# bebop/poly

Measured on AMD Instinct MI355X. Metric: mash.Sketch k-mers hashed/s, higher is better.
Workload: dtype u32

## Files before the change

### poly_amd/csrc/mash_sketch.hip

```cpp
#include <hip/hip_runtime.h>

#include <algorithm>

#include "common.h"
#include "host_pipeline.h"
#include "multi_device.h"
#include <memory>
#include <string>
#include <vector>

#ifndef PH_WPE
#define PH_WPE 6
#endif
#ifndef PH_CAPK
#define PH_CAPK 12u
#endif
#ifndef PH_ABL
#define PH_ABL 0
#endif
#ifndef PH_SELBINS
#define PH_SELBINS 0
#endif
#ifndef PH_SEL_ATOMIC
#define PH_SEL_ATOMIC 0
#endif
#ifndef PH_BS_WIN
#define PH_BS_WIN 4
#endif
#ifndef PH_BS_U
#define PH_BS_U 4
#endif
#ifndef PH_SLAB_SIG
#define PH_SLAB_SIG 6u
#endif
#ifndef PH_SLAB_CW
#define PH_SLAB_CW 6u
#endif
#ifndef PH_SLAB_CF
#define PH_SLAB_CF 0u
#endif
#ifndef PH_SLAB_WPE
#define PH_SLAB_WPE PH_WPE
#endif

namespace polyhip {
namespace k1 {

constexpr int THREADS = 256;
constexpr int WAVES = THREADS / 64;
#ifndef PH_WTW
#define PH_WTW 512
#endif
constexpr int WTW = PH_WTW;
constexpr int TW = WTW * WAVES;
constexpr int GROUPS = WTW / (4 * 64);
constexpr int NB = 2048;
constexpr uint32_t MARK0 = 0xFFFFFFFFu, MARK1 = 0u;
constexpr int GBATCH = 32;
constexpr uint32_t WL_POSITIONAL = 0x80000000u;
constexpr uint32_t C1 = 0xcc9e2d51u, C2 = 0x1b873593u;

__device__ __forceinline__ uint32_t rotl32(uint32_t x, int r) { return (x << r) | (x >> (32 - r)); }

__device__ __forceinline__ uint32_t premix(uint32_t k)
{
    k *= C1;
    k = rotl32(k, 15);
    k *= C2;
    return k;
}

__device__ __forceinline__ uint32_t chain(uint32_t h) { return rotl32(h, 13) * 5u + 0xe6546b64u; }

__device__ __forceinline__ uint32_t fmix32(uint32_t h)
{
    h ^= h >> 16;
    h *= 0x85ebca6bu;
    h ^= h >> 13;
    h *= 0xc2b2ae35u;
    h ^= h >> 16;
    return h;
}

__device__ __forceinline__ uint32_t funnel_bytes(uint32_t hi, uint32_t lo, uint32_t sh)
{
    return __builtin_amdgcn_alignbyte(hi, lo, sh);
}

__device__ __forceinline__ uint32_t wave_incl_scan(uint32_t v)
{
    v += (uint32_t)__builtin_amdgcn_update_dpp(0, (int)v, 0x111, 0xF, 0xF, true);
    v += (uint32_t)__builtin_amdgcn_update_dpp(0, (int)v, 0x112, 0xF, 0xF, true);
    v += (uint32_t)__builtin_amdgcn_update_dpp(0, (int)v, 0x114, 0xF, 0xF, true);
    v += (uint32_t)__builtin_amdgcn_update_dpp(0, (int)v, 0x118, 0xF, 0xF, true);
    v += (uint32_t)__builtin_amdgcn_update_dpp(0, (int)v, 0x142, 0xA, 0xF, false);
    v += (uint32_t)__builtin_amdgcn_update_dpp(0, (int)v, 0x143, 0xC, 0xF, false);
    return v;
}

struct Smem {
    uint32_t *seqb;
    uint32_t *P;
    uint32_t *cand;
    uint32_t *binned;
    uint32_t *misc;
    uint32_t *lut;
};

constexpr uint32_t BIG_BIN = 32;
constexpr uint32_t BIG_LIST_CAP = 512;

template <class Emit>
__device__ __attribute__((noinline)) void rank_big_bins(const uint32_t *__restrict__ binned, const uint32_t *__restrict__ bins,
                                              const uint32_t *__restrict__ biglist, uint32_t nbig, uint32_t s, Emit emit)
{
    const int lane = threadIdx.x & 63, wave = threadIdx.x >> 6;
    const uint64_t below = (1ull << lane) - 1ull;
    for (uint32_t q = wave; q < nbig; q += WAVES) {
        const uint32_t b = biglist[q];
        const uint32_t st = b ? bins[b - 1] : 0u, en = bins[b];
        uint32_t base = st, lastv = 0;
        bool first = true;
        while (base < s && base < en) {
            uint32_t m = 0xFFFFFFFFu;
            bool has = false;
            for (uint32_t x = st + lane; x < en; x += 64) {
                const uint32_t o = binned[x];
                if (first || o > lastv) {
                    m = min(m, o);
                    has = true;
                }
            }
            if (__ballot(has) == 0ull)
                break;
#pragma unroll
            for (int d = 32; d >= 1; d >>= 1)
                m = min(m, (uint32_t)__shfl_xor((int)m, d, 64));
            for (uint32_t x0 = st; x0 < en; x0 += 64) {
                const uint32_t x = x0 + lane;
                const bool eq = x < en && binned[x] == m;
                const uint64_t mask = __ballot(eq);
                const uint32_t pos = base + (uint32_t)__builtin_popcountll(mask & below);
                if (eq && pos < s)
                    emit(pos, m);
                base += (uint32_t)__builtin_popcountll(mask);
            }
            lastv = m;
            first = false;
        }
    }
}

template <class ForEach>
__device__ uint32_t bottom_s(const Smem &sm, uint32_t s, uint32_t tau, uint32_t binned_cap, bool keep_partial,
                             ForEach for_each)
{
    const int tid = threadIdx.x;
    uint32_t *bins = sm.P;
    const int sig = 32 - __builtin_clz(tau | 1u);
    const int shift = sig > 11 ? sig - 11 : 0;
    __syncthreads();

    for (int b = tid; b < NB; b += THREADS)
        bins[b] = 0;
    if (tid == 0)
        sm.misc[8] = 0;
    __syncthreads();
    for_each([&](uint32_t h) {
        if (h <= tau)
            atomicAdd(&bins[h >> shift], 1u);
    });
    __syncthreads();

    {
        uint32_t v[8], sum = 0;
#pragma unroll
        for (int i = 0; i < 8; ++i) {
            v[i] = bins[8 * tid + i];
            sum += v[i];
        }
        uint32_t incl = sum;
#pragma unroll
        for (int d = 1; d < 64; d <<= 1) {
            uint32_t t = __shfl_up(incl, d, 64);
            if ((tid & 63) >= d)
                incl += t;
        }
        if ((tid & 63) == 63)
            sm.misc[4 + (tid >> 6)] = incl;
        __syncthreads();
        uint32_t run = incl - sum;
        for (int w = 0; w < (tid >> 6); ++w)
            run += sm.misc[4 + w];
#pragma unroll
        for (int i = 0; i < 8; ++i) {
            bins[8 * tid + i] = run;
// ... 188 lines not shown
        }
#pragma unroll
        for (int c = 0; c < 4; ++c)
            h[c] = PH_ABL == 3 ? h[c] : fmix32(h[c]);
        emit(4u * (uint32_t)wq, h);
    }
    wave_sync();
}

template <int KS, bool LOCKSTEP, class Before, class EmitFull, class EmitPart>
__device__ __forceinline__ void run_tiles(const Smem &sm, const uint32_t *__restrict__ gdw, uint32_t gsh,
                                          int64_t gbytes, int64_t nwin, uint32_t k, uint32_t n_seq_dw, uint32_t n_P_w,
                                          Before before, EmitFull emit_full, EmitPart emit_part)
{
    const int wave = threadIdx.x >> 6;
    uint32_t *seqb = sm.seqb + wave * n_seq_dw;
    uint32_t *P = sm.P + wave * n_P_w;
    const int64_t stage_bytes = (int64_t)n_seq_dw * 4 + 4;
    auto is_full = [&](int64_t t0) { return (nwin - t0) >= (int64_t)WTW && t0 + stage_bytes <= gbytes; };
    Stager<KS> st;
    const int64_t first = (int64_t)wave * WTW;
    if (first < nwin)
        st.load(gdw, gsh, gbytes, first, n_seq_dw, is_full(first));
    for (int64_t T0 = 0; T0 < nwin; T0 += TW) {
        if (LOCKSTEP)
            before(T0);
        const int64_t t0 = T0 + first;
        if (t0 >= nwin)
            continue;
        const bool full = is_full(t0);
        st.store(seqb, gdw, gsh, gbytes, t0, n_seq_dw, full);
        wave_sync();
        if (t0 + TW < nwin)
            st.load(gdw, gsh, gbytes, t0 + TW, n_seq_dw, is_full(t0 + TW));
        if (full) {
            tile_compute<KS>(seqb, P, sm.lut, k, [&](uint32_t w0, const uint32_t(&h)[4]) { emit_full(t0, w0, h, 4u); });
        } else {
            const uint32_t wl = (uint32_t)((nwin - t0) < (int64_t)WTW ? (nwin - t0) : (int64_t)WTW);
            tile_compute<KS>(seqb, P, sm.lut, k, [&](uint32_t w0, const uint32_t(&h)[4]) {
                emit_part(t0, w0, h, w0 >= wl ? 0u : (wl - w0 < 4u ? wl - w0 : 4u));
            });
        }
    }
}

__device__ __forceinline__ void append4(uint32_t *__restrict__ counter, uint32_t *__restrict__ cand, uint32_t cap,
                                        const uint32_t (&h)[4], uint32_t nvalid, uint32_t tau)
{
    bool a[4];
    uint64_t m[4];
    uint32_t cnt[4], total = 0;
#pragma unroll
    for (int c = 0; c < 4; ++c) {
        a[c] = (PH_ABL == 4 ? h[c] == 12345u : h[c] <= tau) && (uint32_t)c < nvalid;
        m[c] = __ballot(a[c]);
        cnt[c] = (uint32_t)__popcll(m[c]);
        total += cnt[c];
    }
    if (total == 0)
        return;
    uint32_t base = 0;
    if ((threadIdx.x & 63) == 0)
        base = atomicAdd(counter, total);
    base = __builtin_amdgcn_readfirstlane(base);
#pragma unroll
    for (int c = 0; c < 4; ++c) {
        if (a[c]) {
            const uint32_t idx = base + __builtin_amdgcn_mbcnt_hi((uint32_t)(m[c] >> 32),
                                                                  __builtin_amdgcn_mbcnt_lo((uint32_t)m[c], 0u));
            if (idx < cap)
                cand[idx] = h[c];
        }
        base += cnt[c];
    }
}

constexpr int BSU = PH_BS_U;
constexpr uint32_t BS_MARGIN = (PH_BS_WIN + 3u) & ~3u;
#define BS_SYNC()              \
    do {                       \
        if (PH_ABL != 21)      \
            __syncthreads();   \
    } while (0)
template <bool FIN, bool SELB = false>
__device__ void bottom_s_fast(const Smem &sm, uint32_t s, uint32_t tau, uint32_t C, uint32_t nbf_log2,
                              uint32_t *__restrict__ outp, const uint32_t *__restrict__ src, uint32_t first,
                              uint32_t step, uint32_t cnt, uint32_t *__restrict__ selbins = nullptr)
{
    const int tid = threadIdx.x;
    auto fin = [](uint32_t h) { return FIN ? h ^ (h >> 16) : h; };
    uint32_t *bins = sm.P;
    const uint32_t nbf = 1u << nbf_log2;
    const int sig = 32 - __builtin_clz(tau | 1u);
    const int shift = sig > (int)nbf_log2 ? sig - (int)nbf_log2 : 0;
    uint4 *bins4 = reinterpret_cast<uint4 *>(bins);
    const int q4 = (int)(nbf / (4 * THREADS));
    if (!SELB) {
        for (int q = 0; q < q4; ++q)
            bins4[q4 * tid + q] = make_uint4(0, 0, 0, 0);
        if (tid == 0)
            sm.misc[8] = 0;
    }
    if (PH_BS_WIN) {
        if (tid < PH_BS_WIN)
            sm.binned[-1 - tid] = 0u;
        else if (tid < 2 * PH_BS_WIN)
            sm.binned[C + (uint32_t)tid - PH_BS_WIN] = 0xFFFFFFFFu;
    }
    if (!SELB)
        BS_SYNC();
    if (!SELB) {
        for (uint32_t i0 = first; i0 < cnt; i0 += BSU * step) {
            uint32_t h[BSU];
#pragma unroll
            for (int u = 0; u < BSU; ++u)
                h[u] = i0 + u * step < cnt ? fin(src[i0 + u * step]) : 0u;
#pragma unroll
            for (int u = 0; u < BSU; ++u)
                if (i0 + u * step < cnt)
                    atomicAdd(&bins[h[u] >> shift], 1u);
        }
        BS_SYNC();
    }
    {
        uint4 v[2];
        uint32_t sum = 0;
        uint4 *cnt4 = SELB ? reinterpret_cast<uint4 *>(selbins) : bins4;
        for (int q = 0; q < 2; ++q) {
            v[q] = q < q4 ? cnt4[q4 * tid + q] : make_uint4(0, 0, 0, 0);
            if (SELB && q < q4)
                cnt4[q4 * tid + q] = make_uint4(0, 0, 0, 0);
            sum += v[q].x + v[q].y + v[q].z + v[q].w;
        }
        const uint32_t incl = wave_incl_scan(sum);
        if ((tid & 63) == 63)
            sm.misc[4 + (tid >> 6)] = incl;
        BS_SYNC();
        uint32_t run = incl - sum;
        for (int w = 0; w < (tid >> 6); ++w)
            run += sm.misc[4 + w];
        for (int q = 0; q < 2; ++q) {
            if (q < q4) {
                uint4 o;
                o.x = run;
                o.y = o.x + v[q].x;
                o.z = o.y + v[q].y;
                o.w = o.z + v[q].z;
                run = o.w + v[q].w;
                bins4[q4 * tid + q] = o;
                if (max(max(v[q].x, v[q].y), max(v[q].z, v[q].w)) > BIG_BIN) {
                    const uint32_t cnt4[4] = {v[q].x, v[q].y, v[q].z, v[q].w};
#pragma unroll
                    for (int c = 0; c < 4; ++c)
                        if (cnt4[c] > BIG_BIN) {
                            const uint32_t slot = atomicAdd(&sm.misc[8], 1u);
                            if (slot < BIG_LIST_CAP)
                                sm.seqb[slot] = (uint32_t)(4 * (q4 * tid + q) + c);
                        }
                }
            }
        }
    }
    BS_SYNC();
    for (uint32_t i0 = first; i0 < cnt; i0 += BSU * step) {
        uint32_t h[BSU], at[BSU];
#pragma unroll
        for (int u = 0; u < BSU; ++u)
            h[u] = i0 + u * step < cnt ? fin(src[i0 + u * step]) : 0u;
#pragma unroll
        for (int u = 0; u < BSU; ++u)
            if (i0 + u * step < cnt)
                at[u] = atomicAdd(&bins[h[u] >> shift], 1u);
#pragma unroll
        for (int u = 0; u < BSU; ++u)
            if (i0 + u * step < cnt)
                sm.binned[at[u]] = h[u];
    }
    BS_SYNC();
    const uint32_t nbig = sm.misc[8];
    const bool by_waves = nbig <= BIG_LIST_CAP;
    auto rank_in_bin = [&](uint32_t j, uint32_t hv) {
        const uint32_t b = hv >> shift;
        const uint32_t start = b ? bins[b - 1] : 0u, end = bins[b];
        if (start >= s || (by_waves && end - start > BIG_BIN))
            return;
        uint32_t pos = start;
        for (uint32_t x = start; x < end; ++x) {
            const uint32_t o = sm.binned[x];
            pos += (o < hv) || (o == hv && x < j);
        }
        if (pos < s)
            outp[pos] = hv;
    };
#if PH_BS_WIN
    if (PH_ABL != 22) {
        const uint32_t lim = 1u << shift;
        for (uint32_t j = tid; j < C; j += THREADS) {
            const uint32_t *__restrict__ w = sm.binned + j;
            const uint32_t hv = w[0];
            uint32_t pos = j;
            bool far;
            {
                uint32_t l[PH_BS_WIN], r[PH_BS_WIN];
#pragma unroll
                for (int d = 0; d < PH_BS_WIN; ++d) {
                    l[d] = w[-1 - d];
                    r[d] = w[1 + d];
                }
#pragma unroll
                for (int d = 0; d < PH_BS_WIN; ++d) {
                    pos -= l[d] > hv ? 1u : 0u;
                    pos += r[d] < hv ? 1u : 0u;
                }
                far = ((l[PH_BS_WIN - 1] ^ hv) < lim) | ((r[PH_BS_WIN - 1] ^ hv) < lim);
            }
            if (__builtin_expect(far, 0))
                rank_in_bin(j, hv);
            else if (pos < s)
                outp[pos] = hv;
        }
    }
#else
    for (uint32_t j = tid; j < C; j += THREADS)
        rank_in_bin(j, sm.binned[j]);
#endif
    if (by_waves && nbig)
        rank_big_bins(sm.binned, bins, sm.seqb, nbig, s, [outp](uint32_t pos, uint32_t hv) { outp[pos] = hv; });
}

struct ReadView {
    const uint32_t *gdw;
    uint32_t gsh;
    int64_t gbytes, nwin;
};

__device__ __forceinline__ ReadView view(const uint8_t *__restrict__ seqs, const uint64_t *__restrict__ offs,
                                         uint64_t r, uint32_t k)
{
    ReadView v;
    const uint64_t o0 = offs[r], o1 = offs[r + 1];
    const int64_t n = (int64_t)(o1 - o0);
    v.nwin = n - (int64_t)k;
    v.gsh = (uint32_t)((uintptr_t)(seqs + o0) & 3);
    v.gdw = reinterpret_cast<const uint32_t *>(seqs + o0 - v.gsh);
    v.gbytes = n + v.gsh;
    return v;
}

template <int KS>
__global__ __launch_bounds__(THREADS) __attribute__((amdgpu_waves_per_eu(PH_WPE, 8))) void sketch_fast_kernel(const uint8_t *__restrict__ seqs,
                                                             const uint64_t *__restrict__ offs, uint64_t nseq,
                                                             uint32_t k_rt, uint32_t s, uint32_t *__restrict__ out,
                                                             uint32_t n_seq_dw, uint32_t n_P_w, uint32_t n_P,
                                                             uint32_t capf, uint32_t nbf_log2)
{
    extern __shared__ __attribute__((aligned(16))) uint32_t smem_raw[];
    Smem sm;
    sm.seqb = smem_raw;
    sm.P = sm.seqb + WAVES * n_seq_dw;
    sm.cand = sm.P + n_P;
    sm.binned = sm.cand + capf + BS_MARGIN;
    sm.misc = sm.binned + capf + BS_MARGIN;
    sm.lut = sm.misc + 16;

    const uint32_t k = KS > 0 ? (uint32_t)KS : k_rt;
    const int tid = threadIdx.x;
    sm.lut[tid] = premix((uint32_t)tid) ^ k;
    auto nothing = [](int64_t) {};

    for (uint64_t r = blockIdx.x; r < nseq; r += gridDim.x) {
        const ReadView rv = view(seqs, offs, r, k);
        if (rv.nwin <= 0)
            continue;
        uint32_t *__restrict__ outp = out + r * (uint64_t)s;

        if (rv.nwin < (int64_t)s) {
            __syncthreads();
            auto put = [&](int64_t t0, uint32_t w0, const uint32_t(&h)[4], uint32_t nvalid) {
#pragma unroll
                for (int c = 0; c < 4; ++c)
                    if ((uint32_t)c < nvalid)
                        outp[t0 + w0 + c] = h[c];
            };
            run_tiles<KS, false>(sm, rv.gdw, rv.gsh, rv.gbytes, rv.nwin, k, n_seq_dw, n_P_w, nothing, put, put);
            continue;
        }

        uint32_t tau0 = 0xFFFFFFFFu;
        {
            const uint64_t target = (uint64_t)s + 6ull * (uint64_t)__builtin_sqrtf((float)s) + 16ull;
            if ((int64_t)target < rv.nwin)
                tau0 = (uint32_t)((target << 32) / (uint64_t)rv.nwin);
        }
        bool ok = tau0 != 0xFFFFFFFFu || rv.nwin <= (int64_t)capf;
        __syncthreads();
        if (tid == 0)
            sm.misc[0] = 0;
        __syncthreads();
        uint32_t C = 0;
        if (ok) {
            auto keep = [&](int64_t, uint32_t, const uint32_t(&h)[4], uint32_t nvalid) {
                append4(&sm.misc[0], sm.cand, capf, h, nvalid, tau0);
            };
            run_tiles<KS, false>(sm, rv.gdw, rv.gsh, rv.gbytes, rv.nwin, k, n_seq_dw, n_P_w, nothing, keep, keep);
            __syncthreads();
            C = sm.misc[0];
            ok = C >= s && C <= capf;
        }
        if (ok) {
            if (PH_ABL == 5) {
                for (uint32_t i = tid; i < s; i += THREADS)
                    outp[i] = sm.cand[i];
            } else {
                bottom_s_fast<false>(sm, s, tau0, C, nbf_log2, outp, sm.cand, (uint32_t)tid, THREADS, C);
            }
        } else if (tid == 0) {
            outp[0] = MARK0;
            outp[1] = MARK1;
        }
    }
}

template <int KS> struct Slabs {
    static constexpr int NBLK = KS >> 2, TAIL = KS & 3;
    static constexpr int DUPD = NBLK + 2;
    const uint32_t *__restrict__ gdw;
    uint32_t gsh;
    int64_t gbytes;
    uint32_t *__restrict__ seqb;
    uint32_t *__restrict__ P;
    const uint32_t *__restrict__ lut;
    int lane;

    uint32_t u_inside;
    __device__ __forceinline__ void gload(uint32_t u, uint32_t &lo, uint32_t &hi) const
    {
        const uint32_t *__restrict__ slab = gdw + (uint64_t)u * 64;
        hi = 0u;
        if (__builtin_expect(u < u_inside, 1)) {
            lo = slab[lane];
            if (gsh)
                hi = slab[lane + 1];
        } else {
            const int64_t left = gbytes - (int64_t)u * 256;
            lo = (int64_t)lane * 4 < left ? slab[lane] : 0u;
            if (gsh)
                hi = (int64_t)(lane + 1) * 4 < left ? slab[lane + 1] : 0u;
        }
    }

    template <int PAR> __device__ __forceinline__ void stage(uint32_t lo, uint32_t hi) const
    {
        const uint32_t v = gsh ? funnel_bytes(hi, lo, gsh) : lo;
        seqb[1 + 64 * PAR + lane] = v;
        if (PAR == 0) {
            if (lane < DUPD)
                seqb[129 + lane] = v;
        } else if (lane == 63) {
            seqb[0] = v;
        }
    }

    template <int PAR> __device__ __forceinline__ void premix_unit() const
    {
        const uint32_t d0 = seqb[64 * PAR + lane], d1 = seqb[64 * PAR + lane + 1];
        uint4 p;
        p.x = premix(d0);
        p.y = premix(funnel_bytes(d1, d0, 1));
        p.z = premix(funnel_bytes(d1, d0, 2));
        p.w = premix(funnel_bytes(d1, d0, 3));
        uint4 *P4 = reinterpret_cast<uint4 *>(P);
        if (PAR == 0) {
            P4[(lane + 127) & 127] = p;
            if (lane >= 1 && lane <= NBLK)
                P4[127 + lane] = p;
        } else {
            P4[63 + lane] = p;
        }
    }

    template <int PAR> __device__ __forceinline__ void hash(uint32_t (&h)[4]) const
    {
        const uint4 *b = reinterpret_cast<const uint4 *>(P) + 64 * PAR + lane;
        h[0] = h[1] = h[2] = h[3] = 0u;
#pragma unroll
        for (int j = 0; j < (PH_ABL == 16 ? 1 : NBLK); ++j) {
            const uint4 p = b[j];
            h[0] = chain(h[0] ^ p.x);
            h[1] = chain(h[1] ^ p.y);
            h[2] = chain(h[2] ^ p.z);
            h[3] = chain(h[3] ^ p.w);
        }
        const uint32_t *t = seqb + 1 + 64 * PAR + lane + NBLK;
        if (TAIL == 1) {
            const uint32_t tb = t[0];
            uint32_t off[4];
            const uint32_t two = 2u;
            asm("v_lshlrev_b32_sdwa %0, %1, %2 dst_sel:DWORD dst_unused:UNUSED_PAD src0_sel:DWORD src1_sel:BYTE_0" : "=v"(off[0]) : "v"(two), "v"(tb));
            asm("v_lshlrev_b32_sdwa %0, %1, %2 dst_sel:DWORD dst_unused:UNUSED_PAD src0_sel:DWORD src1_sel:BYTE_1" : "=v"(off[1]) : "v"(two), "v"(tb));
            asm("v_lshlrev_b32_sdwa %0, %1, %2 dst_sel:DWORD dst_unused:UNUSED_PAD src0_sel:DWORD src1_sel:BYTE_2" : "=v"(off[2]) : "v"(two), "v"(tb));
            asm("v_lshlrev_b32_sdwa %0, %1, %2 dst_sel:DWORD dst_unused:UNUSED_PAD src0_sel:DWORD src1_sel:BYTE_3" : "=v"(off[3]) : "v"(two), "v"(tb));
#pragma unroll
            for (int c = 0; c < 4; ++c)
                h[c] ^= *reinterpret_cast<const uint32_t *>(reinterpret_cast<const char *>(lut) + off[c]);
        } else if (TAIL) {
            constexpr uint32_t tailmask = 0xFFFFFFFFu >> (32 - 8 * (TAIL ? TAIL : 1));
            const uint32_t d0 = t[0], d1 = t[1];
            h[0] ^= premix(d0 & tailmask) ^ (uint32_t)KS;
            h[1] ^= premix(funnel_bytes(d1, d0, 1) & tailmask) ^ (uint32_t)KS;
            h[2] ^= premix(funnel_bytes(d1, d0, 2) & tailmask) ^ (uint32_t)KS;
            h[3] ^= premix(funnel_bytes(d1, d0, 3) & tailmask) ^ (uint32_t)KS;
        } else {
#pragma unroll
            for (int c = 0; c < 4; ++c)
                h[c] ^= (uint32_t)KS;
        }
#pragma unroll
        for (int c = 0; c < 4; ++c) {
            uint32_t x = h[c];
            if (PH_ABL != 17) {
                x ^= x >> 16;
                x *= 0x85ebca6bu;
                x ^= x >> 13;
            }
            x *= 0xc2b2ae35u;
            h[c] = x;
        }
    }
};

template <bool PARTIAL>
__device__ __forceinline__ void append_own(uint32_t *__restrict__ seg, uint32_t capw, uint32_t &cnt, const uint32_t (&h)[4],
                                           uint32_t nvalid, uint32_t tauq, uint32_t *__restrict__ selbins = nullptr,
                                           uint32_t selshift = 0)
{
    bool a[4];
    uint64_t m[4];
    uint32_t n[4], total = 0;
#pragma unroll
    for (int c = 0; c < 4; ++c) {
        a[c] = h[c] <= tauq && (!PARTIAL || (uint32_t)c < nvalid);
        m[c] = __ballot(a[c]);
        n[c] = (uint32_t)__popcll(m[c]);
        total += n[c];
    }
    uint32_t base = __builtin_amdgcn_readfirstlane(cnt);
    cnt = base + total;
#if PH_SEL_ATOMIC
    {
        uint32_t *ctr = seg + capw;
        uint32_t slot[4];
#pragma unroll
        for (int c = 0; c < 4; ++c)
            if (a[c])
                slot[c] = atomicInc(ctr, capw - 1u);
#pragma unroll
        for (int c = 0; c < 4; ++c)
            if (a[c])
                seg[slot[c]] = h[c];
        return;
    }
#endif
    if (cnt <= capw) {
#pragma unroll
        for (int c = 0; c < 4; ++c) {
            uint32_t *__restrict__ at = seg + base;
            if (a[c]) {
                at[__builtin_amdgcn_mbcnt_hi((uint32_t)(m[c] >> 32), __builtin_amdgcn_mbcnt_lo((uint32_t)m[c], 0u))] = h[c];
                if (PH_SELBINS)
                    atomicAdd(&selbins[h[c] >> selshift], 1u);
            }
            base += n[c];
        }
    }
}

template <int KS>
__device__ __forceinline__ uint32_t run_slabs(const Smem &sm, const ReadView &rv, uint32_t n_seq_dw, uint32_t n_P_w,
                                              uint32_t *__restrict__ seg, uint32_t capw, uint32_t tauq,
                                              uint32_t *__restrict__ selbins = nullptr, uint32_t selshift = 0)
{
    const int wave = __builtin_amdgcn_readfirstlane(threadIdx.x >> 6);
    Slabs<KS> S;
    S.gdw = rv.gdw;
    S.gsh = rv.gsh;
    S.gbytes = rv.gbytes;
    S.seqb = sm.seqb + wave * n_seq_dw;
    S.P = sm.P + wave * n_P_w;
    S.lut = sm.lut;
    S.lane = threadIdx.x & 63;
    const uint32_t nslab = (uint32_t)((rv.nwin + 255) >> 8);
    const uint32_t spw = (nslab + WAVES - 1) / WAVES;
    const uint32_t a = (uint32_t)wave * spw, b = a + spw < nslab ? a + spw : nslab;
    S.u_inside = rv.gbytes >= 65 * 4 ? (uint32_t)(((rv.gbytes >> 2) - 65) >> 6) + 1u : 0u;
    uint32_t cnt = 0;
#if PH_SEL_ATOMIC
    capw -= 1u;
    if (S.lane == 0)
        seg[capw] = 0u;
#endif
    if (a >= b)
        return cnt;
    uint32_t l1, h1;
    S.gload(a, l1, h1);
    if (a & 1) {
        S.template stage<1>(l1, h1);
        wave_sync();
        S.gload(a + 1, l1, h1);
        S.template premix_unit<1>();
    } else {
        S.template stage<0>(l1, h1);
        wave_sync();
        S.gload(a + 1, l1, h1);
        S.template premix_unit<0>();
    }
    for (uint32_t i = a; i < b; ++i) {
        uint32_t h[4];
        if (i & 1) {
            S.template stage<0>(l1, h1);
            wave_sync();
            S.gload(i + 2, l1, h1);
            if (PH_ABL != 15)
                S.template premix_unit<0>();
            wave_sync();
            S.template hash<1>(h);
        } else {
            S.template stage<1>(l1, h1);
            wave_sync();
            S.gload(i + 2, l1, h1);
            if (PH_ABL != 15)
                S.template premix_unit<1>();
            wave_sync();
            S.template hash<0>(h);
        }
        const int64_t left = rv.nwin - ((int64_t)i << 8);
        if (PH_ABL == 11) {
            if ((h[0] ^ h[1] ^ h[2] ^ h[3]) == 0x12345u)
                seg[0] = h[0];
        } else if (__builtin_expect(left >= 256, 1)) {
            append_own<false>(seg, capw, cnt, h, 4u, tauq, selbins, selshift);
        } else {
            const int64_t mine = left - 4 * S.lane;
            append_own<true>(seg, capw, cnt, h, mine <= 0 ? 0u : (mine < 4 ? (uint32_t)mine : 4u), tauq, selbins, selshift);
        }
        wave_sync();
    }
    return cnt;
}

template <int KS>
__global__ __launch_bounds__(THREADS) __attribute__((amdgpu_waves_per_eu(PH_SLAB_WPE, 8))) void sketch_slab_kernel(
    const uint8_t *__restrict__ seqs, const uint64_t *__restrict__ offs, uint64_t nseq, uint32_t s, uint32_t *__restrict__ out,
    uint32_t n_seq_dw, uint32_t n_P_w, uint32_t n_P, uint32_t capw, uint32_t capf, uint32_t nbf_log2)
{
    extern __shared__ __attribute__((aligned(16))) uint32_t smem_raw[];
    Smem sm;
    sm.lut = smem_raw;
    sm.seqb = smem_raw + 256;
    sm.P = sm.seqb + WAVES * n_seq_dw;
    sm.cand = sm.P + n_P;
    sm.binned = sm.cand + WAVES * capw + BS_MARGIN;
    sm.misc = sm.binned + capf + BS_MARGIN;
    constexpr uint32_t k = (uint32_t)KS;
    const int tid = threadIdx.x, wave = __builtin_amdgcn_readfirstlane(tid >> 6);
    sm.lut[tid] = premix((uint32_t)tid) ^ k;
    uint32_t *seg = sm.cand + wave * capw;
    uint32_t *selbins = sm.misc + 16;
    if (PH_SELBINS)
        for (uint32_t b = tid; b < (1u << nbf_log2); b += THREADS)
            selbins[b] = 0u;

    for (uint64_t r = blockIdx.x; r < nseq; r += gridDim.x) {
        const ReadView rv = view(seqs, offs, r, k);
        if (rv.nwin <= 0)
            continue;
        uint32_t *__restrict__ outp = out + r * (uint64_t)s;
        if (rv.nwin < (int64_t)s)
            continue;
        uint32_t tauq = 0xFFFFFFFFu;
        {
            const uint64_t target = (uint64_t)s + (uint64_t)PH_SLAB_SIG * (uint64_t)__builtin_sqrtf((float)s) + 16ull;
            if ((int64_t)target < rv.nwin)
                tauq = (uint32_t)((target << 32) / (uint64_t)rv.nwin) | 0xFFFFu;
        }
        __syncthreads();
        uint32_t selshift = 0;
        if (PH_SELBINS) {
            const int sig = 32 - __builtin_clz(tauq | 1u);
            selshift = sig > (int)nbf_log2 ? (uint32_t)(sig - (int)nbf_log2) : 0u;
            if (tid == 0)
                sm.misc[8] = 0;
        }
        const uint32_t cw = PH_ABL == 14 ? tauq >> 31 : run_slabs<KS>(sm, rv, n_seq_dw, n_P_w, seg, capw, tauq, selbins, selshift);
        if ((tid & 63) == 0)
            sm.misc[10 + wave] = cw;
        __syncthreads();
        if (PH_ABL == 11 || PH_ABL == 12 || PH_ABL == 14) {
            if (sm.misc[10] + sm.misc[11] + sm.misc[12] + sm.misc[13] == 0xFFFFFFF0u)
                outp[0] = cw;
            continue;
        }
        const uint32_t c0 = sm.misc[10], c1 = sm.misc[11], c2 = sm.misc[12], c3 = sm.misc[13];
        const uint32_t C = c0 + c1 + c2 + c3;
        const bool ok = max(max(c0, c1), max(c2, c3)) <= capw - (PH_SEL_ATOMIC ? 1u : 0u) && C >= s && C <= capf;
        if (ok)
            bottom_s_fast<true, PH_SELBINS != 0>(sm, s, tauq, C, nbf_log2, outp, seg, (uint32_t)(tid & 63), 64u, cw, selbins);
        else {
            if (PH_SELBINS)
                for (uint32_t b = tid; b < (1u << nbf_log2); b += THREADS)
                    selbins[b] = 0u;
            if (tid == 0) {
                outp[0] = MARK0;
                outp[1] = MARK1;
            }
        }
    }
}

template <int KS>
__global__ __launch_bounds__(THREADS) void sketch_general_kernel(const uint8_t *__restrict__ seqs,
                                                                const uint64_t *__restrict__ offs, uint32_t k_rt,
                                                                uint32_t s, uint32_t *__restrict__ out,
                                                                uint32_t n_seq_dw, uint32_t n_P_w, uint32_t n_P,
                                                                uint32_t cap, uint64_t nseq, int take_positional)
{
    extern __shared__ __attribute__((aligned(16))) uint32_t smem_raw[];
    Smem sm;
    sm.seqb = smem_raw;
    sm.P = sm.seqb + WAVES * n_seq_dw;
    sm.cand = sm.P + n_P;
    sm.binned = sm.cand + cap;
    sm.misc = sm.binned + cap;
    sm.lut = sm.misc + 16;
    __shared__ uint32_t wl[GBATCH];
    __shared__ uint32_t nwl;

    const uint32_t k = KS > 0 ? (uint32_t)KS : k_rt;
    const int tid = threadIdx.x;
    sm.lut[tid] = premix((uint32_t)tid) ^ k;

    for (uint64_t base = (uint64_t)blockIdx.x * GBATCH; base < nseq; base += (uint64_t)gridDim.x * GBATCH) {
        __syncthreads();
        if (tid == 0)
            nwl = 0;
        __syncthreads();
        {
            const uint64_t r = base + tid;
            if (tid < GBATCH && r < nseq) {
                const int64_t nwin = (int64_t)(offs[r + 1] - offs[r]) - (int64_t)k;
                uint32_t need = 0;
                if (nwin >= (int64_t)s) {
                    const uint32_t *row = out + r * (uint64_t)s;
                    if (row[0] == MARK0 && row[1] == MARK1)
                        need = 1;
                } else if (nwin > 0 && take_positional) {
                    need = 2;
                }
                if (need)
                    wl[atomicAdd(&nwl, 1u)] = (uint32_t)tid | (need == 2 ? WL_POSITIONAL : 0u);
            }
        }
        __syncthreads();
        const uint32_t nredo = nwl;
    for (uint32_t q = 0; q < nredo; ++q) {
        const uint32_t entry = wl[q];
        const uint64_t r = base + (entry & ~WL_POSITIONAL);
        const ReadView rv = view(seqs, offs, r, k);
        uint32_t *__restrict__ outp = out + r * (uint64_t)s;
        __syncthreads();
        if (entry & WL_POSITIONAL) {
            auto put = [&](int64_t t0, uint32_t w0, const uint32_t(&h)[4], uint32_t nvalid) {
#pragma unroll
                for (int c = 0; c < 4; ++c)
                    if ((uint32_t)c < nvalid)
                        outp[t0 + w0 + c] = h[c];
            };
            run_tiles<KS, false>(sm, rv.gdw, rv.gsh, rv.gbytes, rv.nwin, k, n_seq_dw, n_P_w, [](int64_t) {}, put, put);
            continue;
        }
        if (tid == 0) {
            sm.misc[0] = 0;
            sm.misc[1] = 0xFFFFFFFFu;
        }
        __syncthreads();
        auto shrink_shared = [&]() {
            const uint32_t C = sm.misc[0];
            bottom_s(sm, s, sm.misc[1], cap, true, [&](auto f) {
                for (uint32_t i = tid; i < C; i += THREADS)
                    f(sm.cand[i]);
            });
        };
        auto append = [&](int64_t, uint32_t, const uint32_t(&h)[4], uint32_t nvalid) {
            append4(&sm.misc[0], sm.cand, cap, h, nvalid, sm.misc[1]);
        };
        run_tiles<KS, true>(
            sm, rv.gdw, rv.gsh, rv.gbytes, rv.nwin, k, n_seq_dw, n_P_w,
            [&](int64_t) {
// ... 51 lines not shown
    sm.misc = misc;
    sm.lut = nullptr;
    const int tid = threadIdx.x;
    for (uint64_t r = blockIdx.x; r < nseq; r += gridDim.x) {
        const uint64_t o0 = offs[r];
        const int64_t nwin = (int64_t)(offs[r + 1] - o0) - (int64_t)k;
        if (nwin <= 0)
            continue;
        const uint8_t *__restrict__ sp = seqs + o0;
        uint32_t *__restrict__ outp = out + r * (uint64_t)s;
        if (nwin < (int64_t)s) {
            for (int64_t w = tid; w < nwin; w += THREADS)
                outp[w] = murmur3_window(sp + w, k);
            continue;
        }
        __syncthreads();
        if (tid == 0) {
            misc[0] = 0;
            misc[1] = 0xFFFFFFFFu;
        }
        __syncthreads();
        auto shrink = [&]() {
            const uint32_t C = misc[0];
            bottom_s(sm, s, misc[1], cap, true, [&](auto f) {
                for (uint32_t i = tid; i < C; i += THREADS)
                    f(sm.cand[i]);
            });
        };
        for (int64_t base = 0; base < nwin; base += WIDE_ROUND) {
            __syncthreads();
            const bool room = misc[0] + WIDE_ROUND <= cap;
            __syncthreads();
            if (!room)
                shrink();
            const uint32_t tau = misc[1];
#pragma unroll
            for (int c = 0; c < 4; ++c) {
                const int64_t w = base + c * THREADS + tid;
                if (w < nwin) {
                    const uint32_t h = murmur3_window(sp + w, k);
                    if (h <= tau)
                        sm.cand[atomicAdd(&misc[0], 1u)] = h;
                }
            }
        }
        __syncthreads();
        shrink();
        for (uint32_t i = tid; i < s; i += THREADS)
            outp[i] = sm.cand[i];
    }
}

__global__ __launch_bounds__(THREADS) void sketch_tiny_kernel(const uint8_t *__restrict__ seqs,
                                                             const uint64_t *__restrict__ offs, uint64_t nseq, uint32_t k,
                                                             uint32_t s, uint32_t *__restrict__ out,
                                                             unsigned long long *__restrict__ first_panic)
{
    const int tid = threadIdx.x;
    for (uint64_t r = blockIdx.x; r < nseq; r += gridDim.x) {
        const uint64_t o0 = offs[r];
        const int64_t nwin = (int64_t)(offs[r + 1] - o0) - (int64_t)k;
        if (nwin <= 0)
            continue;
        if (s == 0) {
            if (tid == 0)
                atomicMin(first_panic, (unsigned long long)r);
            continue;
        }
        const uint8_t *__restrict__ sp = seqs + o0;
        const uint32_t h0 = murmur3_window(sp, k);
        bool under = false;
        for (int64_t w = 1 + tid; w < nwin && !under; w += THREADS)
            under = murmur3_window(sp + w, k) < h0;
        if (__syncthreads_or(under ? 1 : 0)) {
            if (tid == 0)
                atomicMin(first_panic, (unsigned long long)r);
        } else if (tid == 0) {
            out[r] = h0;
        }
    }
}

struct Launch {
    uint32_t n_seq_dw, n_P_w, n_P, n_P_fast, nbf_log2, nbf_log2_slab, capf, cap, capw, capf_slab;
    size_t smem_fast, smem_general, smem_slab;
};

static Launch plan(uint32_t k, uint32_t s)
{
    Launch L;
    const uint32_t nblk = k / 4;
    L.n_seq_dw = ((WTW / 4 + nblk + 2) + 3u) & ~3u;
    L.n_P_w = WTW + 4 * nblk;
    L.n_P = WAVES * L.n_P_w;
    L.n_P_fast = L.n_P < 1024u ? 1024u : L.n_P;
    L.nbf_log2 = L.n_P_fast >= 2048u ? 11u : 10u;
    if (L.n_P < (uint32_t)NB)
        L.n_P = NB;
    const uint32_t s4 = (s + 3u) & ~3u;
    uint32_t rt = 1;
    while ((uint64_t)rt * rt < s)
        ++rt;
    L.capf = (s4 + PH_CAPK * rt + 64u + 63u) & ~63u;
    L.cap = s4 + TW + 64u;
    const size_t common = (size_t)WAVES * L.n_seq_dw + L.n_P + 16 + 256;
    L.smem_fast = ((size_t)WAVES * L.n_seq_dw + L.n_P_fast + 16 + 256 + 2 * (size_t)L.capf + 2 * BS_MARGIN) * 4;
    if (PH_ABL == 7)
        L.smem_fast = 70 * 1024;
    L.smem_general = (common + 2 * (size_t)L.cap) * 4;
    {
        const uint32_t target = s + PH_SLAB_SIG * rt + 16u;
        const uint32_t exp_w = (target + WAVES - 1) / WAVES;
        uint32_t rw = 1;
        while ((uint64_t)rw * rw < exp_w)
            ++rw;
        L.capw = (exp_w + PH_SLAB_CW * rw + 8u + 63u) & ~63u;
        L.capf_slab = PH_SLAB_CF ? ((target + PH_SLAB_CF * rt + 8u + 63u) & ~63u) : L.capf;
    }
    L.smem_slab = ((size_t)WAVES * L.n_seq_dw + L.n_P_fast + 16 + 256 + (size_t)WAVES * L.capw + (size_t)L.capf_slab + 2 * BS_MARGIN) * 4;
    L.nbf_log2_slab = L.nbf_log2;
    if (PH_SELBINS) {
        L.nbf_log2_slab = PH_SELBINS;
        L.smem_slab += (size_t)4 << PH_SELBINS;
    }
#ifdef PH_LDS_PAD
    L.smem_slab += PH_LDS_PAD;
#endif
    return L;
}

static unsigned persistent_grid(size_t smem, uint64_t n)
{
    const uint64_t per_cu = std::max<uint64_t>(1, std::min<uint64_t>(8, (160 * 1024) / std::max<size_t>(smem, 1)));
    return (unsigned)std::min<uint64_t>(n, 256 * per_cu * 4);
}

template <int KS>
static int launch(const uint8_t *d_seqs, const uint64_t *d_offs, uint64_t n, uint32_t k, uint32_t s,
                  uint32_t *d_out, const Launch &L, hipStream_t st)
{
    auto general = sketch_general_kernel<KS>;
    PH_HIP(hipFuncSetAttribute(reinterpret_cast<const void *>(general), hipFuncAttributeMaxDynamicSharedMemorySize,
                               (int)L.smem_general));
    bool slabs = false;
    if constexpr (KS > 0) {
        slabs = !env_is("POLYHIP_K1_SLABS", '0') && L.smem_slab <= 64 * 1024;
        if (slabs) {
            auto slab = sketch_slab_kernel<KS>;
            PH_HIP(hipFuncSetAttribute(reinterpret_cast<const void *>(slab), hipFuncAttributeMaxDynamicSharedMemorySize,
                                       (int)L.smem_slab));
            hipLaunchKernelGGL(slab, dim3(persistent_grid(L.smem_slab, n)), dim3(THREADS), L.smem_slab, st, d_seqs, d_offs, n, s,
                               d_out, L.n_seq_dw, L.n_P_w, L.n_P_fast, L.capw, L.capf_slab, L.nbf_log2_slab);
        }
    }
    if (!slabs) {
        auto fast = sketch_fast_kernel<KS>;
        PH_HIP(hipFuncSetAttribute(reinterpret_cast<const void *>(fast), hipFuncAttributeMaxDynamicSharedMemorySize,
                                   (int)L.smem_fast));
        hipLaunchKernelGGL(fast, dim3(persistent_grid(L.smem_fast, n)), dim3(THREADS), L.smem_fast, st, d_seqs, d_offs, n,
                           k, s, d_out, L.n_seq_dw, L.n_P_w, L.n_P_fast, L.capf, L.nbf_log2);
    }
    PH_HIP(hipGetLastError());
    const unsigned ggrid = (unsigned)std::min<uint64_t>((n + GBATCH - 1) / GBATCH, persistent_grid(L.smem_general, n));
    hipLaunchKernelGGL(general, dim3(ggrid), dim3(THREADS), L.smem_general, st, d_seqs, d_offs, k, s, d_out, L.n_seq_dw,
                       L.n_P_w, L.n_P, L.cap, n, slabs ? 1 : 0);
    PH_HIP(hipGetLastError());
    return POLYHIP_OK;
}

}
}

using namespace polyhip;

extern "C" {

int polyhip_mash_sketch_batch_dev(const uint8_t *d_seqs, const uint64_t *d_offsets, uint64_t n, uint32_t k,
                                  uint32_t s, uint32_t *d_out, polyhip_stream_t stream)
{
    if (n == 0)
        return POLYHIP_OK;
    PH_REQUIRE(d_seqs && d_offsets && (d_out || s == 0), "polyhip_mash_sketch_batch: null pointer");
    PH_REQUIRE(s <= (1u << 24), "polyhip_mash_sketch_batch: SketchSize %u > 2^24 is not implemented", s);
    hipStream_t st = as_stream(stream);
    if (s < 2) {
        unsigned long long *d_first = nullptr, h_first = ~0ull;
        PH_HIP(hipMallocAsync(reinterpret_cast<void **>(&d_first), sizeof h_first, st));
        StreamFree guard{d_first, st};
        PH_HIP(hipMemsetAsync(d_first, 0xFF, sizeof h_first, st));
        hipLaunchKernelGGL(k1::sketch_tiny_kernel, dim3((unsigned)std::min<uint64_t>(n, 4096)), dim3(k1::THREADS), 0, st, d_seqs,
                           d_offsets, n, k, s, d_out, d_first);
        PH_HIP(hipGetLastError());
        PH_HIP(hipMemcpyAsync(&h_first, d_first, sizeof h_first, hipMemcpyDeviceToHost, st));
        PH_HIP(guard.release());
        PH_HIP(hipStreamSynchronize(st));
        if (h_first != ~0ull)
            return set_error(POLYHIP_ERR_PANIC,
                             "mash.Sketch with SketchSize %u indexes Sketches[-1] on sequence %llu (mash.go:%s): the reference panics",
                             s, h_first + (unsigned long long)md::base().item, s == 0 ? "96" : "98");
        return POLYHIP_OK;
    }
    const k1::Launch L = k1::plan(k <= 4096 ? k : 4096, s <= 8192 ? s : 8192);
    if (s > 8192 || k > 4096 || L.smem_general > 160 * 1024) {
        const uint32_t s4 = (s + 3u) & ~3u;
        const uint32_t cap = 2 * s4 + 2 * k1::WIDE_ROUND;
        const uint64_t per_wg = 2ull * cap * sizeof(uint32_t), budget = 4ull << 30;
        const unsigned grid = (unsigned)std::max<uint64_t>(
            1, std::min<uint64_t>(std::min<uint64_t>(n, s > 16384 ? 256 : 1024), budget / per_wg));
        uint32_t *scratch = nullptr;
        PH_HIP(hipMallocAsync(reinterpret_cast<void **>(&scratch), (size_t)grid * per_wg, st));
        StreamFree guard{scratch, st};
        hipLaunchKernelGGL(k1::sketch_wide_kernel, dim3(grid), dim3(k1::THREADS), 0, st, d_seqs, d_offsets, n, k, s, d_out, scratch,
                           cap);
        PH_HIP(hipGetLastError());
        PH_HIP(guard.release());
        return POLYHIP_OK;
    }
    const uint64_t CHUNK = 1ull << 30;
    for (uint64_t i0 = 0; i0 < n; i0 += CHUNK) {
        const uint64_t m = n - i0 < CHUNK ? n - i0 : CHUNK;
        const uint64_t *offs = d_offsets + i0;
        uint32_t *outp = d_out + i0 * (uint64_t)s;
        int rc;
        switch (k) {
        case 17: rc = k1::launch<17>(d_seqs, offs, m, k, s, outp, L, st); break;
        case 21: rc = k1::launch<21>(d_seqs, offs, m, k, s, outp, L, st); break;
        case 31: rc = k1::launch<31>(d_seqs, offs, m, k, s, outp, L, st); break;
        default: rc = k1::launch<0>(d_seqs, offs, m, k, s, outp, L, st); break;
        }
        if (rc != POLYHIP_OK)
            return rc;
    }
    return POLYHIP_OK;
}

// ... 157 lines not shown
```

Measured before the change: 802.8 billion.

## Pack bottom-s bin counters to 16 bits and alias sort scratch over slab rings

```diff
diff --git a/poly_amd/csrc/mash_sketch.hip b/poly_amd/csrc/mash_sketch.hip
--- a/poly_amd/csrc/mash_sketch.hip
+++ b/poly_amd/csrc/mash_sketch.hip
@@ -17,9 +17,6 @@
 #endif
 #ifndef PH_ABL
 #define PH_ABL 0
-#endif
-#ifndef PH_SELBINS
-#define PH_SELBINS 0
 #endif
 #ifndef PH_SEL_ATOMIC
 #define PH_SEL_ATOMIC 0
@@ -40,7 +37,7 @@
 #define PH_SLAB_CF 0u
 #endif
 #ifndef PH_SLAB_WPE
-#define PH_SLAB_WPE PH_WPE
+#define PH_SLAB_WPE 8
 #endif
 
 namespace polyhip {
@@ -105,13 +102,16 @@
     uint32_t *binned;
     uint32_t *misc;
     uint32_t *lut;
+    uint32_t *bins;
+    uint32_t *biglist;
+    uint32_t listcap;
 };
 
 constexpr uint32_t BIG_BIN = 32;
 constexpr uint32_t BIG_LIST_CAP = 512;
 
-template <class Emit>
-__device__ __attribute__((noinline)) void rank_big_bins(const uint32_t *__restrict__ binned, const uint32_t *__restrict__ bins,
+template <class Bin, class Emit>
+__device__ __attribute__((noinline)) void rank_big_bins(const uint32_t *__restrict__ binned, const Bin *__restrict__ bins,
                                               const uint32_t *__restrict__ biglist, uint32_t nbig, uint32_t s, Emit emit)
 {
     const int lane = threadIdx.x & 63, wave = threadIdx.x >> 6;
@@ -466,83 +466,85 @@
         if (PH_ABL != 21)      \
             __syncthreads();   \
     } while (0)
-template <bool FIN, bool SELB = false>
+template <bool FIN>
 __device__ void bottom_s_fast(const Smem &sm, uint32_t s, uint32_t tau, uint32_t C, uint32_t nbf_log2,
                               uint32_t *__restrict__ outp, const uint32_t *__restrict__ src, uint32_t first,
-                              uint32_t step, uint32_t cnt, uint32_t *__restrict__ selbins = nullptr)
+                              uint32_t step, uint32_t cnt)
 {
     const int tid = threadIdx.x;
     auto fin = [](uint32_t h) { return FIN ? h ^ (h >> 16) : h; };
-    uint32_t *bins = sm.P;
-    const uint32_t nbf = 1u << nbf_log2;
+    uint32_t *bins = sm.bins;
+    const uint16_t *bins16 = reinterpret_cast<const uint16_t *>(bins);
     const int sig = 32 - __builtin_clz(tau | 1u);
     const int shift = sig > (int)nbf_log2 ? sig - (int)nbf_log2 : 0;
-    uint4 *bins4 = reinterpret_cast<uint4 *>(bins);
-    const int q4 = (int)(nbf / (4 * THREADS));
-    if (!SELB) {
-        for (int q = 0; q < q4; ++q)
-            bins4[q4 * tid + q] = make_uint4(0, 0, 0, 0);
-        if (tid == 0)
-            sm.misc[8] = 0;
-    }
+    auto one = [](uint32_t b) { return 1u << ((b & 1u) << 4); };
+    const bool wide = nbf_log2 == 11u;
+    if (wide)
+        reinterpret_cast<uint4 *>(bins)[tid] = make_uint4(0, 0, 0, 0);
+    else
+        reinterpret_cast<uint2 *>(bins)[tid] = make_uint2(0, 0);
+    if (tid == 0)
+        sm.misc[8] = 0;
     if (PH_BS_WIN) {
         if (tid < PH_BS_WIN)
             sm.binned[-1 - tid] = 0u;
         else if (tid < 2 * PH_BS_WIN)
             sm.binned[C + (uint32_t)tid - PH_BS_WIN] = 0xFFFFFFFFu;
     }
-    if (!SELB)
-        BS_SYNC();
-    if (!SELB) {
-        for (uint32_t i0 = first; i0 < cnt; i0 += BSU * step) {
-            uint32_t h[BSU];
-#pragma unroll
-            for (int u = 0; u < BSU; ++u)
-                h[u] = i0 + u * step < cnt ? fin(src[i0 + u * step]) : 0u;
-#pragma unroll
-            for (int u = 0; u < BSU; ++u)
-                if (i0 + u * step < cnt)
-                    atomicAdd(&bins[h[u] >> shift], 1u);
-        }
-        BS_SYNC();
-    }
+    BS_SYNC();
+    for (uint32_t i0 = first; i0 < cnt; i0 += BSU * step) {
+        uint32_t h[BSU];
+#pragma unroll
+        for (int u = 0; u < BSU; ++u)
+            h[u] = i0 + u * step < cnt ? fin(src[i0 + u * step]) : 0u;
+#pragma unroll
+        for (int u = 0; u < BSU; ++u)
+            if (i0 + u * step < cnt) {
+                const uint32_t b = h[u] >> shift;
+                atomicAdd(&bins[b >> 1], one(b));
+            }
+    }
+    BS_SYNC();
     {
-        uint4 v[2];
-        uint32_t sum = 0;
-        uint4 *cnt4 = SELB ? reinterpret_cast<uint4 *>(selbins) : bins4;
-        for (int q = 0; q < 2; ++q) {
-            v[q] = q < q4 ? cnt4[q4 * tid + q] : make_uint4(0, 0, 0, 0);
-            if (SELB && q < q4)
-                cnt4[q4 * tid + q] = make_uint4(0, 0, 0, 0);
-            sum += v[q].x + v[q].y + v[q].z + v[q].w;
+        uint32_t w[4];
+        if (wide) {
+            const uint4 t = reinterpret_cast<const uint4 *>(bins)[tid];
+            w[0] = t.x, w[1] = t.y, w[2] = t.z, w[3] = t.w;
+        } else {
+            const uint2 t = reinterpret_cast<const uint2 *>(bins)[tid];
+            w[0] = t.x, w[1] = t.y, w[2] = 0u, w[3] = 0u;
+        }
+        uint32_t c[8], sum = 0;
+#pragma unroll
+        for (int i = 0; i < 8; ++i) {
+            c[i] = (w[i >> 1] >> (16 * (i & 1))) & 0xFFFFu;
+            sum += c[i];
         }
         const uint32_t incl = wave_incl_scan(sum);
         if ((tid & 63) == 63)
             sm.misc[4 + (tid >> 6)] = incl;
         BS_SYNC();
         uint32_t run = incl - sum;
-        for (int w = 0; w < (tid >> 6); ++w)
-            run += sm.misc[4 + w];
-        for (int q = 0; q < 2; ++q) {
-            if (q < q4) {
-                uint4 o;
-                o.x = run;
-                o.y = o.x + v[q].x;
-                o.z = o.y + v[q].y;
-                o.w = o.z + v[q].z;
-                run = o.w + v[q].w;
-                bins4[q4 * tid + q] = o;
-                if (max(max(v[q].x, v[q].y), max(v[q].z, v[q].w)) > BIG_BIN) {
-                    const uint32_t cnt4[4] = {v[q].x, v[q].y, v[q].z, v[q].w};
-#pragma unroll
-                    for (int c = 0; c < 4; ++c)
-                        if (cnt4[c] > BIG_BIN) {
-                            const uint32_t slot = atomicAdd(&sm.misc[8], 1u);
-                            if (slot < BIG_LIST_CAP)
-                                sm.seqb[slot] = (uint32_t)(4 * (q4 * tid + q) + c);
-                        }
+        for (int w8 = 0; w8 < (tid >> 6); ++w8)
+            run += sm.misc[4 + w8];
+        const uint32_t b0 = (uint32_t)tid << (wide ? 3 : 2);
+#pragma unroll
+        for (int i = 0; i < 4; ++i) {
+            w[i] = run | ((run + c[2 * i]) << 16);
+            run += c[2 * i] + c[2 * i + 1];
+        }
+        if (wide)
+            reinterpret_cast<uint4 *>(bins)[tid] = make_uint4(w[0], w[1], w[2], w[3]);
+        else
+            reinterpret_cast<uint2 *>(bins)[tid] = make_uint2(w[0], w[1]);
+        if (max(max(max(c[0], c[1]), max(c[2], c[3])), max(max(c[4], c[5]), max(c[6], c[7]))) > BIG_BIN) {
+#pragma unroll
+            for (int i = 0; i < 8; ++i)
+                if (c[i] > BIG_BIN) {
+                    const uint32_t slot = atomicAdd(&sm.misc[8], 1u);
+                    if (slot < sm.listcap)
+                        sm.biglist[slot] = b0 + (uint32_t)i;
                 }
-            }
         }
     }
     BS_SYNC();
@@ -553,8 +555,10 @@
             h[u] = i0 + u * step < cnt ? fin(src[i0 + u * step]) : 0u;
 #pragma unroll
         for (int u = 0; u < BSU; ++u)
-            if (i0 + u * step < cnt)
-                at[u] = atomicAdd(&bins[h[u] >> shift], 1u);
+            if (i0 + u * step < cnt) {
+                const uint32_t b = h[u] >> shift;
+                at[u] = (atomicAdd(&bins[b >> 1], one(b)) >> ((b & 1u) << 4)) & 0xFFFFu;
+            }
 #pragma unroll
         for (int u = 0; u < BSU; ++u)
             if (i0 + u * step < cnt)
@@ -562,10 +566,10 @@
     }
     BS_SYNC();
     const uint32_t nbig = sm.misc[8];
-    const bool by_waves = nbig <= BIG_LIST_CAP;
+    const bool by_waves = nbig <= sm.listcap;
     auto rank_in_bin = [&](uint32_t j, uint32_t hv) {
         const uint32_t b = hv >> shift;
-        const uint32_t start = b ? bins[b - 1] : 0u, end = bins[b];
+        const uint32_t start = b ? bins16[b - 1] : 0u, end = bins16[b];
         if (start >= s || (by_waves && end - start > BIG_BIN))
             return;
         uint32_t pos = start;
@@ -609,7 +613,7 @@
         rank_in_bin(j, sm.binned[j]);
 #endif
     if (by_waves && nbig)
-        rank_big_bins(sm.binned, bins, sm.seqb, nbig, s, [outp](uint32_t pos, uint32_t hv) { outp[pos] = hv; });
+        rank_big_bins(sm.binned, bins16, sm.biglist, nbig, s, [outp](uint32_t pos, uint32_t hv) { outp[pos] = hv; });
 }
 
 struct ReadView {
@@ -646,6 +650,9 @@
     sm.binned = sm.cand + capf + BS_MARGIN;
     sm.misc = sm.binned + capf + BS_MARGIN;
     sm.lut = sm.misc + 16;
+    sm.bins = sm.P;
+    sm.biglist = sm.seqb;
+    sm.listcap = BIG_LIST_CAP;
 
     const uint32_t k = KS > 0 ? (uint32_t)KS : k_rt;
     const int tid = threadIdx.x;
@@ -710,13 +717,13 @@
     static constexpr int DUPD = NBLK + 2;
     const uint32_t *__restrict__ gdw;
     uint32_t gsh;
-    int64_t gbytes;
     uint32_t *__restrict__ seqb;
     uint32_t *__restrict__ P;
     const uint32_t *__restrict__ lut;
     int lane;
 
     uint32_t u_inside;
+    uint32_t gb32;
     __device__ __forceinline__ void gload(uint32_t u, uint32_t &lo, uint32_t &hi) const
     {
         const uint32_t *__restrict__ slab = gdw + (uint64_t)u * 64;
@@ -726,10 +733,10 @@
             if (gsh)
                 hi = slab[lane + 1];
         } else {
-            const int64_t left = gbytes - (int64_t)u * 256;
-            lo = (int64_t)lane * 4 < left ? slab[lane] : 0u;
+            const int left = (int)(gb32 - u * 256u);
+            lo = lane * 4 < left ? slab[lane] : 0u;
             if (gsh)
-                hi = (int64_t)(lane + 1) * 4 < left ? slab[lane + 1] : 0u;
+                hi = (lane + 1) * 4 < left ? slab[lane + 1] : 0u;
         }
     }
 
@@ -786,7 +793,7 @@
             asm("v_lshlrev_b32_sdwa %0, %1, %2 dst_sel:DWORD dst_unused:UNUSED_PAD src0_sel:DWORD src1_sel:BYTE_3" : "=v"(off[3]) : "v"(two), "v"(tb));
 #pragma unroll
             for (int c = 0; c < 4; ++c)
-                h[c] ^= *reinterpret_cast<const uint32_t *>(reinterpret_cast<const char *>(lut) + off[c]);
+                h[c] ^= *reinterpret_cast<const __attribute__((address_space(3))) uint32_t *>((uintptr_t)off[c]);
         } else if (TAIL) {
             constexpr uint32_t tailmask = 0xFFFFFFFFu >> (32 - 8 * (TAIL ? TAIL : 1));
             const uint32_t d0 = t[0], d1 = t[1];
@@ -815,8 +822,7 @@
 
 template <bool PARTIAL>
 __device__ __forceinline__ void append_own(uint32_t *__restrict__ seg, uint32_t capw, uint32_t &cnt, const uint32_t (&h)[4],
-                                           uint32_t nvalid, uint32_t tauq, uint32_t *__restrict__ selbins = nullptr,
-                                           uint32_t selshift = 0)
+                                           uint32_t nvalid, uint32_t tauq)
 {
     bool a[4];
     uint64_t m[4];
@@ -849,11 +855,8 @@
 #pragma unroll
         for (int c = 0; c < 4; ++c) {
             uint32_t *__restrict__ at = seg + base;
-            if (a[c]) {
+            if (a[c])
                 at[__builtin_amdgcn_mbcnt_hi((uint32_t)(m[c] >> 32), __builtin_amdgcn_mbcnt_lo((uint32_t)m[c], 0u))] = h[c];
-                if (PH_SELBINS)
-                    atomicAdd(&selbins[h[c] >> selshift], 1u);
-            }
             base += n[c];
         }
     }
@@ -861,14 +864,12 @@
 
 template <int KS>
 __device__ __forceinline__ uint32_t run_slabs(const Smem &sm, const ReadView &rv, uint32_t n_seq_dw, uint32_t n_P_w,
-                                              uint32_t *__restrict__ seg, uint32_t capw, uint32_t tauq,
-                                              uint32_t *__restrict__ selbins = nullptr, uint32_t selshift = 0)
+                                              uint32_t *__restrict__ seg, uint32_t capw, uint32_t tauq)
 {
     const int wave = __builtin_amdgcn_readfirstlane(threadIdx.x >> 6);
     Slabs<KS> S;
     S.gdw = rv.gdw;
     S.gsh = rv.gsh;
-    S.gbytes = rv.gbytes;
     S.seqb = sm.seqb + wave * n_seq_dw;
     S.P = sm.P + wave * n_P_w;
     S.lut = sm.lut;
@@ -877,6 +878,8 @@
     const uint32_t spw = (nslab + WAVES - 1) / WAVES;
     const uint32_t a = (uint32_t)wave * spw, b = a + spw < nslab ? a + spw : nslab;
     S.u_inside = rv.gbytes >= 65 * 4 ? (uint32_t)(((rv.gbytes >> 2) - 65) >> 6) + 1u : 0u;
+    S.gb32 = (uint32_t)rv.gbytes;
+    const uint32_t nfull = (uint32_t)(rv.nwin >> 8), rem = (uint32_t)rv.nwin & 255u;
     uint32_t cnt = 0;
 #if PH_SEL_ATOMIC
     capw -= 1u;
@@ -917,15 +920,14 @@
             wave_sync();
             S.template hash<0>(h);
         }
-        const int64_t left = rv.nwin - ((int64_t)i << 8);
         if (PH_ABL == 11) {
             if ((h[0] ^ h[1] ^ h[2] ^ h[3]) == 0x12345u)
                 seg[0] = h[0];
-        } else if (__builtin_expect(left >= 256, 1)) {
-            append_own<false>(seg, capw, cnt, h, 4u, tauq, selbins, selshift);
+        } else if (__builtin_expect(i < nfull, 1)) {
+            append_own<false>(seg, capw, cnt, h, 4u, tauq);
         } else {
-            const int64_t mine = left - 4 * S.lane;
-            append_own<true>(seg, capw, cnt, h, mine <= 0 ? 0u : (mine < 4 ? (uint32_t)mine : 4u), tauq, selbins, selshift);
+            const int mine = (int)rem - 4 * S.lane;
+            append_own<true>(seg, capw, cnt, h, mine <= 0 ? 0u : (mine < 4 ? (uint32_t)mine : 4u), tauq);
         }
         wave_sync();
     }
@@ -935,24 +937,23 @@
 template <int KS>
 __global__ __launch_bounds__(THREADS) __attribute__((amdgpu_waves_per_eu(PH_SLAB_WPE, 8))) void sketch_slab_kernel(
     const uint8_t *__restrict__ seqs, const uint64_t *__restrict__ offs, uint64_t nseq, uint32_t s, uint32_t *__restrict__ out,
-    uint32_t n_seq_dw, uint32_t n_P_w, uint32_t n_P, uint32_t capw, uint32_t capf, uint32_t nbf_log2)
+    uint32_t n_seq_dw, uint32_t n_P_w, uint32_t n_span, uint32_t capw, uint32_t capf, uint32_t nbf_log2)
 {
     extern __shared__ __attribute__((aligned(16))) uint32_t smem_raw[];
     Smem sm;
     sm.lut = smem_raw;
     sm.seqb = smem_raw + 256;
     sm.P = sm.seqb + WAVES * n_seq_dw;
-    sm.cand = sm.P + n_P;
-    sm.binned = sm.cand + WAVES * capw + BS_MARGIN;
-    sm.misc = sm.binned + capf + BS_MARGIN;
+    sm.bins = sm.seqb;
+    sm.binned = sm.bins + ((1u << nbf_log2) >> 1) + BS_MARGIN;
+    sm.biglist = sm.binned + capf + BS_MARGIN;
+    sm.listcap = (uint32_t)(sm.seqb + n_span - sm.biglist);
+    sm.misc = sm.seqb + n_span;
+    sm.cand = sm.misc + 16;
     constexpr uint32_t k = (uint32_t)KS;
     const int tid = threadIdx.x, wave = __builtin_amdgcn_readfirstlane(tid >> 6);
     sm.lut[tid] = premix((uint32_t)tid) ^ k;
     uint32_t *seg = sm.cand + wave * capw;
-    uint32_t *selbins = sm.misc + 16;
-    if (PH_SELBINS)
-        for (uint32_t b = tid; b < (1u << nbf_log2); b += THREADS)
-            selbins[b] = 0u;
 
     for (uint64_t r = blockIdx.x; r < nseq; r += gridDim.x) {
         const ReadView rv = view(seqs, offs, r, k);
@@ -968,14 +969,7 @@
                 tauq = (uint32_t)((target << 32) / (uint64_t)rv.nwin) | 0xFFFFu;
         }
         __syncthreads();
-        uint32_t selshift = 0;
-        if (PH_SELBINS) {
-            const int sig = 32 - __builtin_clz(tauq | 1u);
-            selshift = sig > (int)nbf_log2 ? (uint32_t)(sig - (int)nbf_log2) : 0u;
-            if (tid == 0)
-                sm.misc[8] = 0;
-        }
-        const uint32_t cw = PH_ABL == 14 ? tauq >> 31 : run_slabs<KS>(sm, rv, n_seq_dw, n_P_w, seg, capw, tauq, selbins, selshift);
+        const uint32_t cw = PH_ABL == 14 ? tauq >> 31 : run_slabs<KS>(sm, rv, n_seq_dw, n_P_w, seg, capw, tauq);
         if ((tid & 63) == 0)
             sm.misc[10 + wave] = cw;
         __syncthreads();
@@ -988,15 +982,10 @@
         const uint32_t C = c0 + c1 + c2 + c3;
         const bool ok = max(max(c0, c1), max(c2, c3)) <= capw - (PH_SEL_ATOMIC ? 1u : 0u) && C >= s && C <= capf;
         if (ok)
-            bottom_s_fast<true, PH_SELBINS != 0>(sm, s, tauq, C, nbf_log2, outp, seg, (uint32_t)(tid & 63), 64u, cw, selbins);
-        else {
-            if (PH_SELBINS)
-                for (uint32_t b = tid; b < (1u << nbf_log2); b += THREADS)
-                    selbins[b] = 0u;
-            if (tid == 0) {
-                outp[0] = MARK0;
-                outp[1] = MARK1;
-            }
+            bottom_s_fast<true>(sm, s, tauq, C, nbf_log2, outp, seg, (uint32_t)(tid & 63), 64u, cw);
+        else if (tid == 0) {
+            outp[0] = MARK0;
+            outp[1] = MARK1;
         }
     }
 }
@@ -1214,7 +1203,7 @@
 }
 
 struct Launch {
-    uint32_t n_seq_dw, n_P_w, n_P, n_P_fast, nbf_log2, nbf_log2_slab, capf, cap, capw, capf_slab;
+    uint32_t n_seq_dw, n_P_w, n_P, n_P_fast, nbf_log2, nbf_log2_slab, capf, cap, capw, capf_slab, n_span;
     size_t smem_fast, smem_general, smem_slab;
 };
 
@@ -1249,12 +1238,13 @@
         L.capw = (exp_w + PH_SLAB_CW * rw + 8u + 63u) & ~63u;
         L.capf_slab = PH_SLAB_CF ? ((target + PH_SLAB_CF * rt + 8u + 63u) & ~63u) : L.capf;
     }
-    L.smem_slab = ((size_t)WAVES * L.n_seq_dw + L.n_P_fast + 16 + 256 + (size_t)WAVES * L.capw + (size_t)L.capf_slab + 2 * BS_MARGIN) * 4;
-    L.nbf_log2_slab = L.nbf_log2;
-    if (PH_SELBINS) {
-        L.nbf_log2_slab = PH_SELBINS;
-        L.smem_slab += (size_t)4 << PH_SELBINS;
-    }
+    L.nbf_log2_slab = 11;
+    {
+        const uint32_t rings = WAVES * (L.n_seq_dw + L.n_P_w);
+        const uint32_t sorted = ((1u << L.nbf_log2_slab) >> 1) + L.capf_slab + 2 * BS_MARGIN + L.capf_slab / (BIG_BIN + 1) + 1;
+        L.n_span = rings > sorted ? rings : sorted;
+    }
+    L.smem_slab = ((size_t)256 + L.n_span + 16 + (size_t)WAVES * L.capw) * 4;
 #ifdef PH_LDS_PAD
     L.smem_slab += PH_LDS_PAD;
 #endif
@@ -1282,7 +1272,7 @@
             PH_HIP(hipFuncSetAttribute(reinterpret_cast<const void *>(slab), hipFuncAttributeMaxDynamicSharedMemorySize,
                                        (int)L.smem_slab));
             hipLaunchKernelGGL(slab, dim3(persistent_grid(L.smem_slab, n)), dim3(THREADS), L.smem_slab, st, d_seqs, d_offs, n, s,
-                               d_out, L.n_seq_dw, L.n_P_w, L.n_P_fast, L.capw, L.capf_slab, L.nbf_log2_slab);
+                               d_out, L.n_seq_dw, L.n_P_w, L.n_span, L.capw, L.capf_slab, L.nbf_log2_slab);
         }
     }
     if (!slabs) {
```

Result: faster. 863.6 billion, median of 6 (+7.6%).
